# swesterfeld/audiowmark

Measured on AMD Instinct MI355X. Metric: audio seconds watermarked+decoded per wall-second (xRT), 44.1 kHz stereo, higher is better.
Workload: dtype f32; 1 GPU; 60 min stereo 44.1 kHz white noise per GPU resident in HBM, add+get incl. payload decode, payload 0123456789abcdef0011223344556677, strength 10; parallelism=1 GPU, patterns=108, payload_matches=104, ranks_seen=1

## Files before the change

audiowmark_amd/csrc/host/capi_kernels.cc:

```cpp
#include "context.hh"
#include "syncfinder.hh"
#include "wmget.hh"
#include "wmspeed.hh"
#include "utils.hh"
#include "wmfile.hh"
#include <atomic>
#include <future>
#include <thread>
#include <algorithm>
#include <cmath>
#include <cstdlib>
#include <cstring>
#include <memory>

using namespace awm;
namespace awm { Key capi_key (const uint8_t key[16]); }
namespace awm { extern int g_key_tables_on_device; int clip_key_tables_check (awm_ctx *ctx, const uint8_t *keys, size_t n_keys, long long mismatch_out[9]); }

namespace {

constexpr int LIMITER_BLOCK = Params::mark_sample_rate * int (Params::limiter_block_size_ms) / 1000;
const float LIMITER_CEILING = float (Params::limiter_ceiling);

constexpr int MAX_FRAMES_PER_BIT = 8;

int
check_ctx (awm_ctx *ctx)
{
  if (!ctx)
    {
      set_error ("null context");
      return AWM_ERR_ARG;
    }
  hipError_t e = hipSetDevice (ctx->device);
  if (e != hipSuccess)
    {
      set_error ("hipSetDevice: " + hip_error_string (e));
      return AWM_ERR_HIP;
    }
  if (params().frames_per_bit < 1 || params().frames_per_bit > MAX_FRAMES_PER_BIT || params().payload_size != 128)
    {
      set_error ("unsupported watermark parameters (frames_per_bit outside 1 .. 8 or a short payload)");
      return AWM_ERR_ARG;
    }
  return 0;
}

#define AWM_ENTER(ctx) \
  awm::ParamsBind params_bind__ ((ctx) ? (ctx)->own_params.get() : nullptr); \
  if (int rc__ = check_ctx (ctx)) return rc__

int
frames_per_span (awm_ctx *ctx, long long n_frames1024, int waves_per_simd = 0)
{
  static int cus = 0;
  if (!cus)
    {
      hipDeviceProp_t prop;
      cus = 256;
      if (hipGetDeviceProperties (&prop, ctx->device) == hipSuccess && prop.multiProcessorCount > 0)
        cus = prop.multiProcessorCount;
    }
  const int capacity = cus * 4 * (waves_per_simd > 0 ? waves_per_simd : awmk::add_mix_waves_per_simd());
  long long best_l = 4, best_cost = -1;
  for (int k = 1; k <= 16; k++)
    {
      long long l = (n_frames1024 + (long long) k * capacity - 1) / ((long long) k * capacity);
      l = std::max<long long> (l, 4);
      const long long cost = k * (l + 2);
      if (best_cost < 0 || cost < best_cost)
        {
          best_cost = cost;
          best_l = l;
        }
    }
  return int (std::min<long long> (best_l, 4096));
}

void
fill_pattern (const ResultSet::Pattern& p, awm_pattern& o)
{
  o.time = p.time;
  o.sync_index = p.sync_score.index;
  o.sync_quality = p.sync_score.quality;
  o.block_type = int (p.sync_score.block_type);
  o.type = int (p.type);
  o.decode_error = p.decode_error;
  o.speed = p.speed;
  o.n_bits = std::min<int> (p.bit_vec.size(), 128);
  for (int b = 0; b < o.n_bits; b++)
    o.bits[b] = p.bit_vec[b];
}

DeviceWav
make_wav (const float *pcm_d, size_t n_frames, int n_channels)
{
  DeviceWav w;
  w.data = pcm_d;
  w.n_frames = n_frames;
  w.n_channels = n_channels;
  w.sample_rate = Params::mark_sample_rate;
  return w;
}
// ... 96 lines not shown
{
  AWM_ENTER (ctx);
  if (!ctx->snr_on)
    {
      set_error ("awm_ctx_snr_end without awm_ctx_snr_begin");
      return AWM_ERR_ARG;
    }
  ctx->snr_on = false;
  double acc[2] = { 0, 0 };
  AWM_HIP_CHECK (hipDeviceSynchronize());
  AWM_HIP_CHECK (hipMemcpy (acc, ctx->ws_snr.ptr, sizeof (acc), hipMemcpyDeviceToHost));
  if (delta_power)
    *delta_power = acc[0];
  if (signal_power)
    *signal_power = acc[1];
  return 0;
}

int
awm_add_mix_d (awm_ctx *ctx, const float *pcm_in_d, float *out_d, size_t n_frames, int n_channels,
               const int8_t *frame_mod, double water_delta, size_t first_frame,
               const float *halo_before_d, const float *halo_after_d,
               float *block_max_d, size_t first_block, size_t n_blocks)
{
  AWM_ENTER (ctx);
  if (!pcm_in_d || !out_d || !frame_mod || n_channels < 1)
    {
      set_error ("awm_add_mix_d: bad argument");
      return AWM_ERR_ARG;
    }
  const size_t table_bytes = 2 * mark_block_frame_count() * Params::n_bands;
  if (int rc = ctx->ws_misc.reserve (table_bytes)) return rc;
  AWM_HIP_CHECK (hipMemcpyAsync (ctx->ws_misc.ptr, frame_mod, table_bytes, hipMemcpyHostToDevice, ctx->stream));
  return add_mix_impl (ctx, pcm_in_d, out_d, n_frames, n_channels, ctx->ws_misc.as<int8_t>(), water_delta, first_frame,
                       halo_before_d, halo_after_d, block_max_d, first_block, n_blocks);
}

int
awm_add_limit_d (awm_ctx *ctx, float *out_d, size_t n_frames, int n_channels, size_t first_sample,
                 const float *block_max_d, size_t first_block, size_t n_blocks)
{
  AWM_ENTER (ctx);
  const size_t tab_entries = awmk::limiter_tab_entries ((long long) n_frames, (long long) first_sample, LIMITER_BLOCK);
  if (int rc = ctx->ws_limit_tab.reserve ((tab_entries + 1) * sizeof (float2))) return rc;
  ProfScope ps (ctx, PROF_LIMITER, double (n_frames) * n_channels * 8.0);
  AWM_HIP_CHECK (awmk::launch_limiter (ctx->stream, out_d, (long long) n_frames, n_channels, (long long) first_sample, block_max_d,
                                       (long long) first_block, (long long) n_blocks, LIMITER_BLOCK, LIMITER_CEILING,
                                       ctx->ws_limit_tab.as<float2>(), tab_entries));
  return 0;
}

static int g_add_slab_mb = 0;
extern "C" void awm_debug_set_add_slab_mb (int mb) { g_add_slab_mb = mb < 0 ? 0 : mb; }

static bool
add_buffers_overlap (const float *in, const float *out, size_t n_values)
{
  const uintptr_t a = reinterpret_cast<uintptr_t> (in), b = reinterpret_cast<uintptr_t> (out), bytes = n_values * sizeof (float);
  return a < b + bytes && b < a + bytes;
}

static int
add_full (awm_ctx *ctx, const float *pcm_in_d, float *out_d, size_t n_frames, int n_channels,
          const int8_t *frame_mod_dev, double water_delta, int use_limiter, WorkLane *lane = nullptr, ReadyMarks *marks = nullptr)
{
  if (!lane)
    lane = ctx;
  if (marks)
    {
      marks->disarm();
      marks->base = out_d;
      marks->n_frames = n_frames;
    }
  hipStream_t st = lane->stream;
  float *block_max = nullptr;
  const size_t n_blocks = n_frames / LIMITER_BLOCK + 2;
  if (use_limiter)
    {
      if (int rc = lane->ws_block_max.reserve (n_blocks * sizeof (float))) return rc;
      block_max = lane->ws_block_max.as<float>();
      unsigned int bits;
      std::memcpy (&bits, &LIMITER_CEILING, sizeof (bits));
      AWM_HIP_CHECK (awmk::launch_fill_u32 (st, reinterpret_cast<unsigned int *> (block_max), bits, n_blocks));
    }
  const size_t FRAME = Params::frame_size;
  size_t slab = g_add_slab_mb ? (size_t (g_add_slab_mb) << 20) / (n_channels * sizeof (float)) / FRAME * FRAME : 0;
  if (!use_limiter || pcm_in_d == out_d || slab < 64 * FRAME || n_frames < 2 * slab)
    slab = 0;
  if (slab)
    {
      const size_t tab_entries = awmk::limiter_tab_entries ((long long) n_frames, 0, LIMITER_BLOCK);
      if (int rc = lane->ws_limit_tab.reserve ((tab_entries + 1) * sizeof (float2))) return rc;
      const size_t n_slabs = n_frames / slab;
      size_t limited = 0;
      for (size_t i = 0; i < n_slabs; i++)
        {
          const size_t a = i * slab, b = i + 1 == n_slabs ? n_frames : a + slab;
          if (int rc = add_mix_impl (ctx, pcm_in_d + a * n_channels, out_d + a * n_channels, b - a, n_channels, frame_mod_dev, water_delta,
                                     a / FRAME, a ? pcm_in_d + (a - FRAME) * n_channels : nullptr, b < n_frames ? pcm_in_d + b * n_channels : nullptr,
                                     block_max, 0, n_blocks, lane))
            return rc;
          const size_t upto = b == n_frames ? n_frames : (b / LIMITER_BLOCK >= 1 ? (b / LIMITER_BLOCK - 1) * size_t (LIMITER_BLOCK) : 0);
          if (upto > limited)
            {
              ProfScope ps (ctx, PROF_LIMITER, double (upto - limited) * n_channels * 8.0, st);
              AWM_HIP_CHECK (awmk::launch_limiter (st, out_d + limited * n_channels, (long long) (upto - limited), n_channels, (long long) limited, block_max, 0,
                                                   (long long) n_blocks, LIMITER_BLOCK, LIMITER_CEILING, lane->ws_limit_tab.as<float2>(), tab_entries));
              limited = upto;
            }
        }
      return 0;
    }
  if (int rc = add_mix_impl (ctx, pcm_in_d, out_d, n_frames, n_channels, frame_mod_dev, water_delta, 0, nullptr, nullptr,
                             block_max, 0, n_blocks, lane))
    return rc;
  std::vector<size_t> ends;
  if (marks)
    for (const ChunkRange& c : plan_chunks (n_frames, n_channels))
      {
        size_t e = std::min (n_frames, (c.first_frame + c.n_frames + LIMITER_BLOCK - 1) / LIMITER_BLOCK * size_t (LIMITER_BLOCK));
        if (e < n_frames && n_frames - e < size_t (LIMITER_BLOCK))
          e = n_frames;
        if (ends.empty() || e > ends.back())
          ends.push_back (e);
      }
// ... 614 lines not shown
  std::vector<size_t> idx (index, index + n_blocks);
  std::vector<std::vector<float>> raw;
  std::vector<char> okv;
  if (int rc = block_soft_bits (ctx, kt, make_wav (pcm_d, n_frames, n_channels), idx, raw, okv))
    return rc;
  const size_t n_bits = mark_data_frame_count() / params().frames_per_bit;
  for (size_t i = 0; i < n_blocks; i++)
    {
      ok[i] = okv[i];
      if (okv[i])
        std::copy (raw[i].begin(), raw[i].end(), out + i * n_bits);
      else
        std::fill (out + i * n_bits, out + (i + 1) * n_bits, 0.f);
    }
  return 0;
}

int
awm_viterbi_decode (awm_ctx *ctx, int block_type, const float *soft, size_t coded_len, size_t n, int *bits_out, float *error_out)
{
  AWM_ENTER (ctx);
  if (block_type < 0 || block_type > 2)
    return AWM_ERR_ARG;
  std::vector<std::vector<float>> in (n);
  for (size_t i = 0; i < n; i++)
    in[i].assign (soft + i * coded_len, soft + (i + 1) * coded_len);
  std::vector<std::vector<int>> bits;
  std::vector<float> errors;
  if (int rc = viterbi_decode (ctx, ConvBlockType (block_type), in, bits, errors))
    return rc;
  for (size_t i = 0; i < n; i++)
    {
      std::copy (bits[i].begin(), bits[i].end(), bits_out + i * bits[i].size());
      error_out[i] = errors[i];
    }
  return 0;
}

int
awm_add_watermark_d (awm_ctx *ctx, const uint8_t key[16], const char *payload_hex, const float *pcm_in_d, float *out_d,
                     size_t n_frames, int n_channels, int sample_rate)
{
  AWM_ENTER (ctx);
  if (n_channels >= 1 && add_buffers_overlap (pcm_in_d, out_d, n_frames * size_t (n_channels)))
    {
      set_error ("awm_add_watermark_d: the output overlaps the input");
      return AWM_ERR_ARG;
    }
  FrameModTable *fm = ctx->get_frame_mod (capi_key (key), payload_hex ? payload_hex : "");
  if (!fm)
    return AWM_ERR_ARG;
  if (sample_rate != Params::mark_sample_rate)
    return add_full_rate (ctx, pcm_in_d, out_d, n_frames, n_channels, fm->dev.as<int8_t>(), params().water_delta, !params().test_no_limiter, sample_rate);
  return add_full (ctx, pcm_in_d, out_d, n_frames, n_channels, fm->dev.as<int8_t>(), params().water_delta, !params().test_no_limiter);
}

static int g_add_payloads_fused = 1, g_add_payloads_fused_in_use = 0;
extern "C" void awm_debug_set_add_payloads_fused (int on) { g_add_payloads_fused = on; }
extern "C" int  awm_debug_add_payloads_fused_in_use (void) { return g_add_payloads_fused_in_use; }
extern "C" int  awm_debug_add_payloads_tile (void) { return awmk::ADD_MULTI_TILE; }

int
awm_add_watermark_payloads_d (awm_ctx *ctx, const uint8_t key[16], const char *const *payload_hex, size_t n_payloads,
                              const float *pcm_in_d, float *const *out_d, size_t n_frames, int n_channels, int sample_rate)
{
  AWM_ENTER (ctx);
  g_add_payloads_fused_in_use = 0;
  if (!n_payloads || !n_frames)
    return 0;
  if (!key || !payload_hex || !pcm_in_d || !out_d || n_channels < 1)
    {
      set_error ("awm_add_watermark_payloads_d: bad argument");
      return AWM_ERR_ARG;
    }
  if (ctx->snr_on)
    {
      set_error ("awm_add_watermark_payloads_d: not available while the SNR meter is armed (awm_ctx_snr_begin)");
      return AWM_ERR_ARG;
    }
  const size_t n_values = n_frames * size_t (n_channels);
  auto overlap = [n_values] (const float *a, const float *b) { return a < b + n_values && b < a + n_values; };
  for (size_t p = 0; p < n_payloads; p++)
    {
      if (!payload_hex[p] || !out_d[p])
        {
          set_error (string_printf ("awm_add_watermark_payloads_d: null pointer at index %zu", p));
          return AWM_ERR_ARG;
        }
      if (parse_payload (payload_hex[p]).empty())
        {
          set_error (string_printf ("awm_add_watermark_payloads_d: cannot parse payload '%s' at index %zu", payload_hex[p], p));
          return AWM_ERR_ARG;
        }
      if (overlap (out_d[p], pcm_in_d))
        {
          set_error (string_printf ("awm_add_watermark_payloads_d: output %zu overlaps the input", p));
          return AWM_ERR_ARG;
        }
      for (size_t q = 0; q < p; q++)
        if (overlap (out_d[p], out_d[q]))
          {
            set_error (string_printf ("awm_add_watermark_payloads_d: outputs %zu and %zu overlap", q, p));
            return AWM_ERR_ARG;
          }
    }
  const Key k = capi_key (key);
  const double water_delta = params().water_delta;
// ... 636 lines not shown
  };
  hipEvent_t ev_up[2] = { nullptr, nullptr };
  struct EvGuard { hipEvent_t (&ev)[2]; ~EvGuard() { for (hipEvent_t e : ev) if (e) (void) hipEventDestroy (e); } } guard { ev_up };
  for (auto& e : ev_up)
    AWM_HIP_CHECK (hipEventCreateWithFlags (&e, hipEventDisableTiming));
  std::vector<hipEvent_t> lane_done (2 * size_t (n_lanes), nullptr);
  struct DoneGuard { std::vector<hipEvent_t>& ev; ~DoneGuard() { for (hipEvent_t e : ev) if (e) (void) hipEventDestroy (e); } } done_guard { lane_done };
  for (auto& e : lane_done)
    AWM_HIP_CHECK (hipEventCreateWithFlags (&e, hipEventDisableTiming));
  int rc = 0, last_half = -1;
  std::future<bool> next_built;
  struct FutureGuard { std::future<bool>& f; ~FutureGuard() { if (f.valid()) f.wait(); } } future_guard { next_built };
  for (size_t s0 = 0, sidx = 0; s0 < n_clips && !rc; s0 += SUPER, sidx++)
    {
      const size_t sn = std::min (SUPER, n_clips - s0);
      const int half = int (sidx & 1);
      const bool built = next_built.valid() ? next_built.get() : build_super (s0, half);
      if (!built)
        {
          set_error ("frame_mod table of unexpected size");
          return AWM_ERR_GENERIC;
        }
      if (s0 + SUPER < n_clips)
        {
          if (sidx >= 1)
            AWM_HIP_CHECK (hipEventSynchronize (ev_up[half ^ 1]));
          next_built = std::async (std::launch::async, build_super, s0 + SUPER, half ^ 1);
        }
      int8_t *dev = ctx->ws_keytab.as<int8_t>() + size_t (half) * SUPER * table_bytes;
      if (sidx >= 2)
        for (int i = 1; i < n_lanes; i++)
          AWM_HIP_CHECK (hipStreamWaitEvent (ctx->stream, lane_done[size_t (half) * n_lanes + i], 0));
      AWM_HIP_CHECK (hipMemcpyAsync (dev, pin_base + size_t (half) * SUPER * table_bytes, sn * table_bytes, hipMemcpyHostToDevice, ctx->stream));
      AWM_HIP_CHECK (hipEventRecord (ev_up[half], ctx->stream));
      for (int i = 1; i < n_lanes; i++)
        AWM_HIP_CHECK (hipStreamWaitEvent (lanes[i]->stream, ev_up[half], 0));
      for (size_t i = 0; i < sn && !rc; i++)
        rc = add_full (ctx, pcm_in_d[s0 + i], out_d[s0 + i], n_frames[s0 + i], n_channels, dev + i * table_bytes, params().water_delta,
                       !params().test_no_limiter, lanes[(s0 + i) % n_lanes]);
      for (int i = 1; i < n_lanes && !rc; i++)
        AWM_HIP_CHECK (hipEventRecord (lane_done[size_t (half) * n_lanes + i], lanes[i]->stream));
      last_half = half;
    }
  if (last_half >= 0)
    AWM_HIP_CHECK (hipEventSynchronize (ev_up[last_half]));
  for (int i = 1; i < n_lanes; i++)
    {
      AWM_HIP_CHECK (hipEventRecord (lanes[i]->ev_sync, lanes[i]->stream));
      AWM_HIP_CHECK (hipStreamWaitEvent (ctx->stream, lanes[i]->ev_sync, 0));
    }
  return rc;
}

int
awm_get_watermark_d (awm_ctx *ctx, const uint8_t key[16], const float *pcm_d, size_t n_frames, int n_channels,
                     size_t max_out, awm_pattern *out)
{
  AWM_ENTER (ctx);
  ResultSet rs;
  if (int rc = get_watermark_device (ctx, { capi_key (key) }, make_wav (pcm_d, n_frames, n_channels), rs))
    return rc;
  for (size_t i = 0; i < rs.patterns.size() && i < max_out; i++)
    fill_pattern (rs.patterns[i], out[i]);
  return int (rs.patterns.size());
}


int
awm_get_watermark_keys_d (awm_ctx *ctx, const uint8_t *keys, int n_keys, const float *pcm_d, size_t n_frames, int n_channels,
                          size_t max_out, awm_pattern *out, int *key_of_pattern)
{
  AWM_ENTER (ctx);
  if (n_keys < 0 || (n_keys && !keys) || (max_out && !out))
    {
      set_error ("awm_get_watermark_keys_d: bad argument");
      return AWM_ERR_ARG;
    }
  const std::vector<Key> list = key_list_from (keys, n_keys);
  ResultSet rs;
  if (int rc = get_watermark_device (ctx, list, make_wav (pcm_d, n_frames, n_channels), rs))
    return rc;
  return fill_patterns_keys (rs, list, max_out, out, key_of_pattern);
}

int
awm_get_watermark_batch_d (awm_ctx *ctx, const uint8_t key[16], size_t n_clips, const float *const *pcm_d, const size_t *n_frames,
                           int n_channels, int n_threads, size_t max_out_per_clip, awm_pattern *out, int *n_out)
{
  AWM_ENTER (ctx);
  if (n_clips && (!pcm_d || !n_frames || !n_out || (max_out_per_clip && !out)))
    {
      set_error ("awm_get_watermark_batch_d: bad argument");
      return AWM_ERR_ARG;
    }
  std::vector<DeviceWav> clips;
  for (size_t i = 0; i < n_clips; i++)
    clips.push_back (make_wav (pcm_d[i], n_frames[i], n_channels));
  std::vector<ResultSet> sets;
  if (int rc = get_watermark_batch_device (ctx, { capi_key (key) }, clips, sets, n_threads))
    return rc;
  for (size_t i = 0; i < n_clips; i++)
    {
      n_out[i] = int (sets[i].patterns.size());
      for (size_t j = 0; j < sets[i].patterns.size() && j < max_out_per_clip; j++)
        fill_pattern (sets[i].patterns[j], out[i * max_out_per_clip + j]);
    }
  return 0;
}

int
awm_get_watermark_batch_keys_d (awm_ctx *ctx, const uint8_t *keys, size_t n_clips, const float *const *pcm_d, const size_t *n_frames,
                                int n_channels, int n_threads, size_t max_out_per_clip, awm_pattern *out, int *n_out)
{
  AWM_ENTER (ctx);
  if (n_clips && (!keys || !pcm_d || !n_frames || !n_out || (max_out_per_clip && !out)))
    {
      set_error ("awm_get_watermark_batch_keys_d: bad argument");
      return AWM_ERR_ARG;
    }
  std::vector<DeviceWav> clips;
  for (size_t i = 0; i < n_clips; i++)
    clips.push_back (make_wav (pcm_d[i], n_frames[i], n_channels));
  const std::vector<Key> clip_keys = key_list_from (keys, int (n_clips));
  std::vector<ResultSet> sets;
  if (int rc = get_watermark_batch_device (ctx, {}, clips, sets, n_threads, &clip_keys))
// ... 379 lines not shown
```

audiowmark_amd/csrc/host/capi_shard.cc:

```cpp
#include "context.hh"
#include "wmget.hh"
#include "utils.hh"
#include <algorithm>
#include <condition_variable>
#include <cstring>
#include <mutex>
#include <thread>

namespace awm {
Key capi_key (const uint8_t key[16]);
int sharded_plan_c (const uint64_t *span_frames, int world, size_t max_out, int *chunk, int *rank, uint64_t *first_sf, uint64_t *n_sf);
int sharded_add (awm_ctx *ctx, const Key& key, const std::string& payload_hex, const float *pcm_in, float *out, int C,
                 const uint64_t *span_frames, const awm_comm *comm);
int sharded_get (awm_ctx *ctx, const Key& key, const float *pcm, int C, const uint64_t *span_frames, const awm_comm *comm, ResultSet& result);
}

using namespace awm;

namespace {

int
enter (awm_ctx *ctx, const awm_comm *comm, const uint64_t *span_frames, int n_channels)
{
  if (!ctx || !comm || !span_frames || n_channels < 1 || comm->world < 1 || comm->rank < 0 || comm->rank >= comm->world
      || !comm->exchange_d || !comm->exchange_h || !comm->all_reduce_max_u32_d)
    {
      set_error ("awm_sharded_*: bad argument");
      return AWM_ERR_ARG;
    }
  if (hipSetDevice (ctx->device) != hipSuccess)
    {
      set_error ("hipSetDevice failed");
      return AWM_ERR_HIP;
    }
  if (params().frames_per_bit < 1 || params().frames_per_bit > 8 || params().payload_size != 128)
    {
      set_error ("unsupported watermark parameters (frames_per_bit outside 1 .. 8 or a short payload)");
      return AWM_ERR_ARG;
    }
  return 0;
}

void
fill_c_pattern (const ResultSet::Pattern& p, awm_pattern& o)
{
  o.time = p.time;
  o.sync_index = p.sync_score.index;
  o.sync_quality = p.sync_score.quality;
  o.block_type = int (p.sync_score.block_type);
  o.type = int (p.type);
  o.decode_error = p.decode_error;
  o.speed = p.speed;
  o.n_bits = std::min<int> (int (p.bit_vec.size()), 128);
  for (int b = 0; b < o.n_bits; b++)
    o.bits[b] = p.bit_vec[b];
}


struct LocalWorld
{
  int world;
  std::mutex mutex;
  std::condition_variable cond;
  int arrived = 0;
  unsigned long generation = 0;
  bool failed = false;
  struct Post { std::vector<const void *> ptr; std::vector<size_t> bytes; std::vector<int> to; bool device = false; };
  std::vector<Post> posts;
  std::vector<std::vector<uint32_t>> reduce;
  std::vector<int> device_of;
  explicit LocalWorld (int n) : world (n), posts (n), reduce (n), device_of (n, 0), active (n) {}
  int active;
  void
  barrier()
  {
    std::unique_lock<std::mutex> lock (mutex);
    const unsigned long gen = generation;
    arrived++;
    if (arrived >= active)
      {
        arrived = 0;
        generation++;
// ... 393 lines not shown
```

audiowmark_amd/csrc/host/capi_tables.cc:

```cpp
#include "context.hh"
#include "utils.hh"
#include "wmspeed.hh"
#include "random.hh"
#include <cstring>
#include <memory>

using namespace awm;

static Key
key_from_bytes (const uint8_t key[16])
{
  Key k;
  k.set_raw (key);
  return k;
}

namespace awm { Key capi_key (const uint8_t key[16]) { return key_from_bytes (key); } }

extern "C" {

int
awm_tab_up_down (const uint8_t key[16], int stream, int frame, int up[30], int down[30])
{
  UpDownGen gen (key_from_bytes (key), Random::Stream (stream));
// ... 208 lines not shown
      return AWM_ERR_ARG;
    }
  if (!(p->water_delta >= 0) || p->payload_size < 1 || p->frames_per_bit < 1 || p->get_n_best < 1 || !(p->get_chunk_size > 0))
    {
      set_error ("awm_params: value out of range");
      return AWM_ERR_ARG;
    }
  v.water_delta = p->water_delta;
  v.mix = p->mix != 0;
  v.hard = p->hard != 0;
  v.strict = p->strict != 0;
  v.snr = p->snr != 0;
  v.payload_size = size_t (p->payload_size);
  v.frames_per_bit = p->frames_per_bit;
  v.sync_threshold2 = p->sync_threshold2;
  v.get_n_best = p->get_n_best;
  v.get_chunk_size = p->get_chunk_size;
  v.detect_speed = p->detect_speed != 0;
  v.detect_speed_patient = p->detect_speed_patient != 0;
  v.try_speed = p->try_speed;
  v.test_speed = p->test_speed;
  v.test_cut = p->test_cut;
  v.test_no_sync = p->test_no_sync != 0;
  v.test_no_limiter = p->test_no_limiter != 0;
  v.test_truncate = p->test_truncate;
  return 0;
}

void
awm_params_init (awm_params *p)
{
  if (p)
    params_to_c (ParamValues(), p);
}

int
awm_set_global_params (const awm_params *p)
{
  ParamValues v = global_params();
  if (int rc = params_from_c (p, v))
    return rc;
  global_params() = v;
  return 0;
}

int
awm_ctx_set_params (awm_ctx *ctx, const awm_params *p)
{
  if (!ctx)
    {
      set_error ("null context");
      return AWM_ERR_ARG;
    }
  if (!p)
    {
      ctx->own_params.reset();
      return 0;
    }
  auto v = std::make_unique<ParamValues> (ctx->own_params ? *ctx->own_params : global_params());
  if (int rc = params_from_c (p, *v))
    return rc;
  ctx->own_params = std::move (v);
  return 0;
}

int
awm_ctx_get_params (const awm_ctx *ctx, awm_params *out)
{
  if (!out)
    return AWM_ERR_ARG;
  params_to_c (ctx && ctx->own_params ? *ctx->own_params : global_params(), out);
  return 0;
}

void
awm_set_quiet (int quiet)
{
  set_log_level (quiet ? Log::WARNING : Log::INFO);
}

}
```

audiowmark_amd/csrc/host/context.cc:

```cpp
#include "context.hh"
#include <algorithm>
#include <atomic>
#include <chrono>
#include <cstdlib>
#include "utils.hh"
#include <cmath>
#include <cstring>

namespace awm {

static thread_local std::string g_last_error;
void set_error (const std::string& msg) { g_last_error = msg; }
const std::string& last_error() { return g_last_error; }
std::string hip_error_string (hipError_t e) { return std::string (hipGetErrorName (e)) + " (" + hipGetErrorString (e) + ")"; }

static std::atomic<long>   g_dev_allocs { 0 }, g_pin_allocs { 0 };
static std::atomic<double> g_dev_alloc_ms { 0.0 }, g_pin_alloc_ms { 0.0 };
static void
note_alloc (std::atomic<long>& count, std::atomic<double>& ms, std::chrono::steady_clock::time_point t0)
{
  const double dt = std::chrono::duration<double, std::milli> (std::chrono::steady_clock::now() - t0).count();
  count.fetch_add (1, std::memory_order_relaxed);
  double cur = ms.load (std::memory_order_relaxed);
  while (!ms.compare_exchange_weak (cur, cur + dt, std::memory_order_relaxed))
// ... 654 lines not shown
  ctx->tabs.tw512d = reinterpret_cast<const double2 *> (ctx->tab_slide.as<double>() + off_tw512d);
  ctx->tabs.slide32 = reinterpret_cast<const float2 *> (ctx->tab_slide.as<double>() + off_slide32);
  if (int rc = upload (ctx->tab_mem, blob.data(), blob.size() * sizeof (float), ctx->stream))
    return rc;
  const float *base = ctx->tab_mem.as<float>();
  ctx->tabs.tw512 = reinterpret_cast<const float2 *> (base + off_tw512);
  ctx->tabs.tw1024 = reinterpret_cast<const float2 *> (base + off_tw1024);
  ctx->tabs.window = base + off_win;
  ctx->tabs.synth = base + off_synth;
  if (awmk::probe_dependent_launch_us (ctx->stream) < 0 && hipStreamSynchronize (ctx->stream) != hipSuccess)
    {
      set_error ("awm_ctx_create: the device does not complete work on the context's stream");
      return AWM_ERR_HIP;
    }
  *ctx_out = ctx.release();
  return 0;
}

int
awm_ctx_set_chunk_lanes (awm_ctx *ctx, int n_lanes)
{
  if (!ctx || n_lanes < 1)
    return AWM_ERR_ARG;
  ctx->chunk_lanes = std::min (n_lanes, awm::CHUNK_LANES);
  return 0;
}

int
awm_ctx_warm_up (awm_ctx *ctx, int detect_speed, int file_level)
{
  if (!ctx)
    return AWM_ERR_ARG;
  AWM_HIP_CHECK (hipSetDevice (ctx->device));
  const int lanes = std::max (1, std::min (ctx->chunk_lanes, awm::CHUNK_LANES)) * (detect_speed ? 2 : 1);
  for (int i = 0; i < lanes && i < awm::MAX_LANES; i++)
    if (!ctx->lane (i))
      {
        awm::set_error ("cannot create a work lane (stream)");
        return AWM_ERR_HIP;
      }
  if (file_level && !ctx->get_copy_stream())
    {
      awm::set_error ("cannot create the copy stream");
      return AWM_ERR_HIP;
    }
  return 0;
}

int
awm_ctx_trim (awm_ctx *ctx)
{
  if (!ctx)
    return AWM_ERR_ARG;
  AWM_HIP_CHECK (hipSetDevice (ctx->device));
  AWM_HIP_CHECK (hipStreamSynchronize (ctx->stream));
  for (auto& l : ctx->extra_lanes)
    if (l)
      {
        if (l->stream)
          AWM_HIP_CHECK (hipStreamSynchronize (l->stream));
        l->release_lane();
      }
  if (ctx->copy_stream)
    AWM_HIP_CHECK (hipStreamSynchronize (ctx->copy_stream));
  ctx->release_lane();
  ctx->file_staging.release();
  awm::speed_workspace_free (ctx);
  ctx->ws_add_batch.release();
  ctx->pin_add_batch.release();
  ctx->ws_merge_soft.release();
  ctx->ws_rate_a.release();
  ctx->ws_rate_b.release();
  ctx->ws_rate_c.release();
  for (awm_ctx *h : ctx->helpers)
    if (h && h != ctx)
      if (int rc = awm_ctx_trim (h)) return rc;
  return 0;
}

void
awm_ctx_destroy (awm_ctx *ctx)
{
  if (!ctx)
    return;
  (void) hipSetDevice (ctx->device);
  (void) hipStreamSynchronize (ctx->stream);
  for (auto& kt : ctx->key_tables)
    release_key_tables (*kt);
  for (auto& t : ctx->frame_mod_tables)
    t->dev.release();
  for (auto& t : ctx->resample_tables)
    t->ctab.release();
  awm::speed_workspace_free (ctx);
  ctx->ws_snr.release();
  ctx->ws_add_batch.release();
  ctx->pin_add_batch.release();
  if (ctx->ev_add_batch)
    (void) hipEventDestroy (ctx->ev_add_batch);
  ctx->ev_add_batch = nullptr;
  ctx->ws_merge_soft.release();
  for (hipEvent_t e : ctx->merge_events)
    if (e)
      (void) hipEventDestroy (e);
  ctx->merge_events.clear();
  ctx->ws_rate_a.release();
  ctx->ws_rate_b.release();
  ctx->ws_rate_c.release();
  ctx->tab_mem.release();
  ctx->tab_slide.release();
  for (auto& l : ctx->extra_lanes)
    if (l)
      {
        if (l->stream)
          (void) hipStreamSynchronize (l->stream);
        l->release_lane();
        if (l->own_stream && l->stream)
          (void) hipStreamDestroy (l->stream);
      }
  ctx->release_lane();
  if (ctx->copy_stream)
    (void) hipStreamSynchronize (ctx->copy_stream);
  ctx->file_staging.release();
  ctx->ready.release();
  if (ctx->copy_stream)
    (void) hipStreamDestroy (ctx->copy_stream);
  if (ctx->own_stream && ctx->stream)
    (void) hipStreamDestroy (ctx->stream);
  delete ctx;
}

int awm_ctx_device (const awm_ctx *ctx) { return ctx ? ctx->device : -1; }

int
awm_ctx_synchronize (awm_ctx *ctx)
{
  if (!ctx)
    return AWM_ERR_ARG;
  AWM_HIP_CHECK (hipStreamSynchronize (ctx->stream));
  return 0;
}

void *awm_ctx_stream (awm_ctx *ctx) { return ctx ? (void *) ctx->stream : nullptr; }

int
awm_ctx_set_stream (awm_ctx *ctx, void *hip_stream)
{
  if (!ctx)
    return AWM_ERR_ARG;
  AWM_HIP_CHECK (hipStreamSynchronize (ctx->stream));
  if (ctx->own_stream && ctx->stream)
    (void) hipStreamDestroy (ctx->stream);
  ctx->stream = (hipStream_t) hip_stream;
  ctx->own_stream = false;
  return 0;
}

}
```

audiowmark_amd/csrc/host/context.hh:

```
#pragma once
#include <condition_variable>
#include <mutex>
#include <hip/hip_runtime.h>
#include <map>
#include <mutex>
#include <memory>
#include <string>
#include <vector>
#include "../hip/kernels.hh"
#include "wmcommon.hh"

namespace awm { void set_error (const std::string& msg); const std::string& last_error(); std::string hip_error_string (hipError_t e); }

#define AWM_HIP_CHECK(expr) \
  do { hipError_t e__ = (expr); if (e__ != hipSuccess) { awm::set_error (std::string (#expr) + ": " + awm::hip_error_string (e__)); return AWM_ERR_HIP; } } while (0)

namespace awm {

inline void
cpu_relax()
{
  for (int k = 0; k < 48; k++)
    __builtin_ia32_pause();
}
// ... 74 lines not shown
  int        slice_want_n = 0;
  const int *want_of_slice (int i) const { return slice_want_flat ? slice_want_flat + size_t (i) * slice_want_n : slice_want[i].data(); }
  int        want_rows_of_slices() const { return slice_want_flat ? slice_want_n : int (slice_want[0].size()); }
};

struct ClipKeyHost
{
  std::vector<unsigned>      chains;
  std::vector<int>           row_frames;
  std::vector<int>           want;
  std::vector<int>           perm;
  std::vector<unsigned char> pos;
  MixTable                   mix;
  std::vector<int>           inv_order;
};
ClipKeyHost build_clip_key_host (const Key& key);

struct ResampleTable
{
  int       rate_in = 0, rate_out = 0;
  int       hl = 0, np = 0, step = 0;
  DevBuffer ctab;
};

std::vector<float> zita_table (double frel, unsigned hl, unsigned np);
int upload_sync (DevBuffer& buf, const void *src, size_t bytes, hipStream_t st);

struct SpeedWorkspace;
struct SpeedScratch;
struct WorkLane;
void speed_scratch_free (WorkLane *lane);
} struct awm_ctx; namespace awm {
void speed_workspace_free (awm_ctx *ctx);

struct FileStaging
{
  static constexpr int RING = 4;
  PinnedBuffer in_host[RING], out_host[RING];
  DevBuffer    in_dev[RING], out_dev[RING];
  DevBuffer    pcm;
  bool         keep = false;
  size_t       kept_values = 0;
  int          kept_channels = 0, kept_rate = 0;
  hipEvent_t   in_copied[RING] = {}, in_used[RING] = {}, out_encoded[RING] = {}, out_copied[RING] = {};
  bool         have_events = false;
  bool         ensure_events();
  void         release();
};

struct ReadyMarks
{
  const float *base = nullptr;
  size_t       n_frames = 0;
  bool         armed = false;
  std::vector<std::pair<size_t, hipEvent_t>> marks;
  std::vector<hipEvent_t> pool;
  size_t       used = 0;
  hipEvent_t   next_event();
  bool         live = false, live_done = false;
  std::mutex   mu;
  std::condition_variable cv;
  void         disarm() { armed = false; live = live_done = false; marks.clear(); used = 0; base = nullptr; n_frames = 0; }
  void         release();
};

struct FrameModTable
{
  std::vector<unsigned char> key;
  std::string payload;
  bool        mix = true;
  int         frames_per_bit = 2;
  unsigned long last_use = 0;
  DevBuffer   dev;
};

}

namespace awm {
enum ProfId { PROF_ADD_MIX, PROF_LIMITER, PROF_SYNC_DB, PROF_SYNC_SCAN, PROF_LOCAL_MEAN, PROF_REFINE_DB, PROF_REFINE_SCAN,
              PROF_BLOCK_DB, PROF_SOFT_BITS, PROF_VITERBI, PROF_STFT,
              PROF_RESAMPLE, PROF_RESAMPLE_VAR, PROF_SPEED_MAGS, PROF_SPEED_COMPARE, PROF_KEYTAB, PROF_ADD_MIX_MULTI, PROF_COUNT };
struct ProfPending { int id; hipEvent_t start, stop; };
}

namespace awm {
struct WorkLane
{
  hipStream_t    stream = nullptr;
  bool           own_stream = false;
  DevBuffer ws_db, ws_block_db, ws_have, ws_q, ws_raw, ws_mean, ws_misc, ws_refine, ws_refine_have, ws_soft,
            ws_viterbi, ws_viterbi_in, ws_viterbi_bits, ws_viterbi_err, ws_viterbi_sync, ws_block_max, ws_clip, ws_idx, ws_limit_tab, ws_jobs, ws_group, ws_keytab, ws_keytab_aux, ws_keytab_scratch;
  DevBuffer ws_shard_edge, ws_shard_tail, ws_shard_q;
  PinnedBuffer pin_refine_in[2], pin_refine_q[2], pin_peaks, pin_blocks, pin_jobs, pin_bits, pin_small, pin_group, pin_shard, pin_shard_up, pin_keytab;
  hipEvent_t   ev_refine[2] = { nullptr, nullptr };
  hipEvent_t   ev_sync = nullptr;
  SpeedScratch *speed_scratch = nullptr;
  double       prof_live_fraction = 1.0;
  unsigned int *viterbi_sync (size_t n_decodes);
  void release_lane();
};
constexpr int MAX_LANES = 16;
constexpr int CHUNK_LANES = 4;
}

struct awm_ctx : awm::WorkLane
{
  int            device = -1;
  awmk::DevTables tabs {};
  awm::DevBuffer tab_mem, tab_slide;

  std::vector<std::unique_ptr<awm::KeyTables>>     key_tables;
  std::vector<std::unique_ptr<awm::FrameModTable>> frame_mod_tables;
  std::vector<std::unique_ptr<awm::ResampleTable>> resample_tables;
  awm::ResampleTable *get_resample_table (int rate_in, int rate_out);
  awm::DevBuffer ws_rate_a, ws_rate_b, ws_rate_c;
// ... 69 lines not shown
```

audiowmark_amd/csrc/host/wmget.cc:

```cpp
#include "wmget.hh"
#include "wmdecode.hh"
#include "wmspeed.hh"
#include <atomic>
#include <future>
#include <chrono>
#include <memory>
#include <thread>
#include "utils.hh"
#include <algorithm>
#include <cmath>
#include <map>

namespace awm {
int g_key_tables_on_device = 1;


std::vector<float>
normalize_soft_bits (const std::vector<float>& soft_bits)
{
  std::vector<float> norm;
  norm.reserve (soft_bits.size());
  if (params().hard)
    {
      for (float v : soft_bits)
// ... 457 lines not shown
  }
};

}

void
combine_blocks (const std::vector<PatternRawBits>& raw_blocks, const DeviceWav& wav, size_t chunk, std::vector<PendingDecode>& pending)
{
  const BlockList list { raw_blocks, (long long) (mark_block_frame_count() * Params::frame_size) };
  for (size_t pos = 0; pos < raw_blocks.size(); pos++)
    {
      const PatternRawBits& b = raw_blocks[pos];
      if (b.block_type != ConvBlockType::b)
        continue;
      const size_t partner = list.nearest (0, pos, ConvBlockType::a, (long long) b.index - list.block_len, Params::frame_size / 2);
      if (partner == NO_BLOCK)
        continue;
      const PatternRawBits& a = raw_blocks[partner];
      const SyncFinder::Score score { b.index, (a.quality + b.quality) / 2, ConvBlockType::ab };
      pending.push_back ({ ConvBlockType::ab, 1, { { a.slot, 0 }, { b.slot, 1 } }, 0, 0, double (b.index) / wav.sample_rate, score,
                           ResultSet::Type::BLOCK, chunk });
    }
  std::vector<size_t> best;
  float best_sum = 0;
  for (size_t start = 0; start < raw_blocks.size(); start++)
    {
      std::vector<size_t> chain = list.chain_from (start);
      const float sum = list.quality_sum (chain);
      if (sum > best_sum)
        {
          best = std::move (chain);
          best_sum = sum;
        }
    }
  if (best.size() < 2)
    return;
  PendingDecode all { ConvBlockType::ab, 2, {}, 0, 0, 0.0, { 0, 0, ConvBlockType::a }, ResultSet::Type::ALL, chunk };
  for (size_t pos : best)
    {
      const PatternRawBits& blk = raw_blocks[pos];
      const int ab = blk.block_type == ConvBlockType::b;
      all.src.push_back ({ blk.slot, ab });
      (ab ? all.norm1 : all.norm0)++;
      all.score.quality += blk.quality;
    }
  all.score.quality /= all.norm0 + all.norm1;
  pending.push_back (std::move (all));
}

int g_merge_decodes = 0;
extern "C" void awm_debug_set_merge_decodes (int on) { g_merge_decodes = on; }
int g_chunk_stagger = -1;
extern "C" void awm_debug_set_chunk_stagger (int on) { g_chunk_stagger = on; }
int g_speed_overlap = 1;
extern "C" void awm_debug_set_speed_overlap (int on) { g_speed_overlap = on; }
namespace {

int
block_decoder_run (awm_ctx *ctx, WorkLane *home, bool spread, const std::vector<Key>& key_list, const DeviceWav& stream,
                   const std::vector<ChunkRange>& chunks, const std::vector<ResultSet *>& result_sets, double speed,
                   std::string *debug_sync_first_chunk, int lane_base = 0)
{
  const size_t count = mark_block_frame_count();
  std::vector<SyncFinder::Score> first_scores;
  const int n_lanes = !spread ? 1 : int (std::min<size_t> (chunks.size(), size_t (std::max (1, std::min (ctx->chunk_lanes, CHUNK_LANES)))));
  std::vector<WorkLane *> lanes;
  if (!spread)
    lanes.push_back (home);
  else
    for (int i = 0; i < std::max (n_lanes, 1); i++)
      {
        WorkLane *l = ctx->lane (lane_base + i);
        if (!l)
          {
            set_error ("cannot create a work lane (stream)");
            return AWM_ERR_HIP;
          }
        lanes.push_back (l);
      }
  ReadyMarks *marks = (spread && lane_base == 0 && lanes.size() > 1 && ctx->ready.armed && ctx->ready.base == stream.data
                       && ctx->ready.n_frames == stream.n_frames && (ctx->ready.live || !ctx->ready.marks.empty())) ? &ctx->ready : nullptr;
  if (marks && !marks->live)
    std::rotate (lanes.begin(), lanes.begin() + 1, lanes.end());
  else if (lanes.size() > 1 && lane_base == 0)
    {
      if (!ctx->ev_sync)
        AWM_HIP_CHECK (hipEventCreateWithFlags (&ctx->ev_sync, hipEventDisableTiming));
      AWM_HIP_CHECK (hipEventRecord (ctx->ev_sync, ctx->stream));
      for (size_t i = 1; i < lanes.size(); i++)
        AWM_HIP_CHECK (hipStreamWaitEvent (lanes[i]->stream, ctx->ev_sync, 0));
    }
  auto wait_for_mark = [&] (WorkLane *lane, size_t last_sample_plus_one) -> int {
    if (!marks)
      return 0;
    if (marks->live)
      {
        std::unique_lock<std::mutex> lock (marks->mu);
        marks->cv.wait (lock, [&] { return marks->live_done || (!marks->marks.empty() && marks->marks.back().first >= last_sample_plus_one); });
        hipEvent_t ev = nullptr;
        for (const auto& m : marks->marks)
          if (m.first >= last_sample_plus_one)
            {
              ev = m.second;
              break;
            }
        if (!ev && !marks->marks.empty())
          ev = marks->marks.back().second;
        lock.unlock();
        if (ev)
          AWM_HIP_CHECK (hipStreamWaitEvent (lane->stream, ev, 0));
        return 0;
      }
    if (lane->stream == ctx->stream)
      return 0;
    for (const auto& m : marks->marks)
      if (m.first >= last_sample_plus_one)
        {
          AWM_HIP_CHECK (hipStreamWaitEvent (lane->stream, m.second, 0));
          return 0;
        }
    AWM_HIP_CHECK (hipStreamWaitEvent (lane->stream, marks->marks.back().second, 0));
    return 0;
  };
  struct LaneDrain
  {
    const std::vector<WorkLane *>& lanes;
    bool ok = false;
    ~LaneDrain()
    {
      if (!ok)
        for (WorkLane *l : lanes)
          (void) hipStreamSynchronize (l->stream);
    }
  } drain { lanes };
  auto chunk_wav = [&] (size_t c) {
    DeviceWav cw = stream;
// ... 1334 lines not shown
```

include/awm_hip.h:

```cpp
#ifndef AWM_HIP_H
#define AWM_HIP_H

#include <stddef.h>
#include <stdint.h>

#ifdef __cplusplus
extern "C" {
#endif

#define AWM_ERR_GENERIC    (-1)
#define AWM_ERR_NO_DEVICE  (-2)
#define AWM_ERR_ARG        (-3)
#define AWM_ERR_HIP        (-4)
#define AWM_ERR_IO         (-5)

#define AWM_FRAME_SIZE      1024
#define AWM_N_BANDS         81
#define AWM_BLOCK_FRAMES    2226
#define AWM_SOFT_BITS       858

typedef struct awm_ctx awm_ctx;

const char *awm_last_error (void);
const char *awm_version (void);
// ... 154 lines not shown
                     const uint64_t *span_frames, size_t max_out, awm_pattern *out);

int awm_multi_add_watermark_batch_d (awm_ctx *const *ctxs, int n_ctx, const int *ctx_of_clip, const uint8_t *keys, const uint8_t *one_key,
                                     const char *payload_hex, size_t n_clips, const float *const *pcm_in_d, float *const *out_d,
                                     const size_t *n_frames, int n_channels);
int awm_multi_get_watermark_batch_d (awm_ctx *const *ctxs, int n_ctx, const int *ctx_of_clip, const uint8_t *keys, const uint8_t *one_key,
                                     size_t n_clips, const float *const *pcm_d, const size_t *n_frames, int n_channels,
                                     size_t max_out_per_clip, awm_pattern *out, int *n_out);

int awm_ctx_set_helpers (awm_ctx *ctx, awm_ctx *const *helpers, int n_helpers);

void awm_set_speed_params (int detect_speed, int detect_speed_patient, double try_speed, double test_speed);
size_t awm_resample_ratio_frames (size_t n_frames, int n_channels, int rate, double ratio, double max_in_seconds);
int awm_resample_ratio_d (awm_ctx *ctx, const float *pcm_in_d, size_t n_frames, int n_channels, int rate, double ratio,
                          double max_in_seconds, float *out_d, size_t n_out_frames);
int awm_detect_speed_d (awm_ctx *ctx, const uint8_t key[16], const float *pcm_d, size_t n_frames, int n_channels, int rate,
                        int patient, double *speed_out, double *quality_out);
int awm_speed_clip_location_d (awm_ctx *ctx, const uint8_t key[16], const float *pcm_d, size_t n_frames, int n_channels, int rate,
                               double seconds, int candidates, double *location);
int awm_speed_mags_d (awm_ctx *ctx, const uint8_t key[16], const float *pcm_d, size_t n_frames, int n_channels, int rate,
                      double clip_location, double center, double seconds, size_t max_rows, float *out);
int awm_speed_scan_d (awm_ctx *ctx, const uint8_t key[16], const float *pcm_d, size_t n_frames, int n_channels, int rate,
                      double clip_location, double seconds, double step, int n_steps, int n_center_steps,
                      const double *speeds, int n_speeds, size_t max_out, double *out_speed, double *out_quality);

int    awm_speed_select_n_best (double *speed, double *quality, int count, int n);
double awm_speed_smooth_best (const double *speed, const double *quality, int count, double step, double distance);
size_t awm_speed_clip_positions (const uint8_t key[16], size_t n_values, size_t max_out, uint64_t *positions);
int    awm_speed_clip_candidates (const uint8_t key[16], const float *hashed_values, size_t n, int candidates, double *locations);

void awm_debug_set_viterbi_super (int on);
void awm_debug_set_viterbi_persistent (int on);
double awm_debug_dependent_launch_us (void);
int  awm_debug_viterbi_one_launch_in_use (void);
void awm_debug_set_sliding3 (int on);
void awm_debug_set_refine_form (int form);
int  awm_debug_refine_form (void);
void awm_debug_set_k4s_ablate (int flags);
int  awm_debug_sync_db_sliding_d (awm_ctx *ctx, const float *pcm_d, size_t n_frames, int n_channels, const long long *base_d, size_t n_streams,
                                  int count, int ld, float *out_d);
void awm_debug_set_soft_bits_generic (int on);
void awm_debug_set_chunk_stagger (int mode);
void awm_debug_set_resample_phase (int on);
void awm_debug_set_get_overlap (int on);
void awm_debug_set_speed_compare_wide (int on);
void awm_debug_set_speed_compare_fold (int on);
void awm_debug_set_resample_var_mode (int mode);
void awm_debug_set_speed_overlap (int on);
int  awm_debug_frame_mod_tables_d (awm_ctx *ctx, const uint8_t *keys, size_t n_keys, const char *payload_hex, int8_t *tables_out);
int  awm_debug_clip_key_tables_check_d (awm_ctx *ctx, const uint8_t *keys, size_t n_keys, long long mismatch_out[9]);
void awm_debug_set_key_tables_on_device (int on);
void awm_debug_set_merge_decodes (int on);
void awm_debug_set_add_batched (int on);
void awm_debug_set_add_slab_mb (int mb);
void awm_debug_set_add_payloads_fused (int on);
int  awm_debug_add_payloads_fused_in_use (void);
int  awm_debug_add_payloads_tile (void);
void awm_debug_set_fft_pair (int on);
void awm_debug_set_clip_poison (int on);
void awm_debug_set_clip_pad_margin (int frames);
void awm_debug_set_staged_threads (int n);
void awm_debug_clip_key_timing (double us_out[3]);
double awm_debug_time_group_key_tables (int n_keys, int threads);
void awm_debug_set_group_fallback (int on);
void awm_debug_alloc_stats (long *dev_allocs, double *dev_ms, long *pinned_allocs, double *pinned_ms);
void awm_debug_file_timing (double ms_out[8]);
void awm_debug_set_io_flags (int flags);

void awm_set_io_threads (int n);

void awm_set_quiet (int quiet);

void awm_set_params (double water_delta, int mix, int frames_per_bit, int test_no_limiter,
                     double sync_threshold2, int n_best, double chunk_size_min);
typedef struct
{
  size_t struct_size;
  double water_delta;
  int    mix;
  int    hard;
  int    strict;
  int    snr;
  int    payload_size;
  int    frames_per_bit;
  double sync_threshold2;
  int    get_n_best;
  double get_chunk_size;
  int    detect_speed, detect_speed_patient;
  double try_speed, test_speed;
  int    test_cut, test_no_sync, test_no_limiter, test_truncate;
} awm_params;
void awm_params_init (awm_params *p);
int  awm_set_global_params (const awm_params *p);
int  awm_ctx_set_params (awm_ctx *ctx, const awm_params *p);
int  awm_ctx_get_params (const awm_ctx *ctx, awm_params *out);

int  awm_ctx_snr_begin (awm_ctx *ctx);
int  awm_ctx_snr_end (awm_ctx *ctx, double *signal_power, double *delta_power);

#ifdef __cplusplus
}
#endif
#endif
```

Before: 751,700 xRT.

## Hand per-chunk ready marks from add_watermark to a following get

```diff
diff --git a/audiowmark_amd/csrc/host/capi_kernels.cc b/audiowmark_amd/csrc/host/capi_kernels.cc
--- a/audiowmark_amd/csrc/host/capi_kernels.cc
+++ b/audiowmark_amd/csrc/host/capi_kernels.cc
@@ -46,9 +46,12 @@
   return 0;
 }
 
-#define AWM_ENTER(ctx) \
+#define AWM_ENTER_KEEP_MARKS(ctx) \
   awm::ParamsBind params_bind__ ((ctx) ? (ctx)->own_params.get() : nullptr); \
   if (int rc__ = check_ctx (ctx)) return rc__
+#define AWM_ENTER(ctx) \
+  AWM_ENTER_KEEP_MARKS (ctx); \
+  (ctx)->ready.drop_add_marks()
 
 int
 frames_per_span (awm_ctx *ctx, long long n_frames1024, int waves_per_simd = 0)
@@ -251,6 +254,8 @@
 
 static int g_add_slab_mb = 0;
 extern "C" void awm_debug_set_add_slab_mb (int mb) { g_add_slab_mb = mb < 0 ? 0 : mb; }
+static int g_add_marks = 1;
+extern "C" void awm_debug_set_add_marks (int on) { g_add_marks = on; }
 
 static bool
 add_buffers_overlap (const float *in, const float *out, size_t n_values)
@@ -270,6 +275,7 @@
       marks->disarm();
       marks->base = out_d;
       marks->n_frames = n_frames;
+      marks->n_channels = n_channels;
     }
   hipStream_t st = lane->stream;
   float *block_max = nullptr;
@@ -990,7 +996,12 @@
     return AWM_ERR_ARG;
   if (sample_rate != Params::mark_sample_rate)
     return add_full_rate (ctx, pcm_in_d, out_d, n_frames, n_channels, fm->dev.as<int8_t>(), params().water_delta, !params().test_no_limiter, sample_rate);
-  return add_full (ctx, pcm_in_d, out_d, n_frames, n_channels, fm->dev.as<int8_t>(), params().water_delta, !params().test_no_limiter);
+  const bool hand_over = g_add_marks && !g_add_slab_mb && n_frames > 0 && plan_chunks (n_frames, n_channels).size() > 1;
+  const int rc = add_full (ctx, pcm_in_d, out_d, n_frames, n_channels, fm->dev.as<int8_t>(), params().water_delta, !params().test_no_limiter, nullptr,
+                           hand_over ? &ctx->ready : nullptr);
+  if (rc)
+    ctx->ready.disarm();
+  return rc;
 }
 
 static int g_add_payloads_fused = 1, g_add_payloads_fused_in_use = 0;
@@ -1733,11 +1744,28 @@
   return rc;
 }
 
+extern "C++" {
+namespace {
+struct MarksUse
+{
+  awm_ctx *ctx;
+  MarksUse (awm_ctx *c, const float *pcm_d, size_t n_frames, int n_channels) : ctx (c)
+  {
+    ReadyMarks& rm = ctx->ready;
+    if (!(rm.armed && !rm.live && rm.base == pcm_d && rm.n_frames == n_frames && rm.n_channels == n_channels))
+      rm.disarm();
+  }
+  ~MarksUse() { ctx->ready.disarm(); }
+};
+}
+}
+
 int
 awm_get_watermark_d (awm_ctx *ctx, const uint8_t key[16], const float *pcm_d, size_t n_frames, int n_channels,
                      size_t max_out, awm_pattern *out)
 {
-  AWM_ENTER (ctx);
+  AWM_ENTER_KEEP_MARKS (ctx);
+  MarksUse marks_use (ctx, pcm_d, n_frames, n_channels);
   ResultSet rs;
   if (int rc = get_watermark_device (ctx, { capi_key (key) }, make_wav (pcm_d, n_frames, n_channels), rs))
     return rc;
@@ -1751,7 +1779,8 @@
 awm_get_watermark_keys_d (awm_ctx *ctx, const uint8_t *keys, int n_keys, const float *pcm_d, size_t n_frames, int n_channels,
                           size_t max_out, awm_pattern *out, int *key_of_pattern)
 {
-  AWM_ENTER (ctx);
+  AWM_ENTER_KEEP_MARKS (ctx);
+  MarksUse marks_use (ctx, pcm_d, n_frames, n_channels);
   if (n_keys < 0 || (n_keys && !keys) || (max_out && !out))
     {
       set_error ("awm_get_watermark_keys_d: bad argument");
diff --git a/audiowmark_amd/csrc/host/capi_shard.cc b/audiowmark_amd/csrc/host/capi_shard.cc
--- a/audiowmark_amd/csrc/host/capi_shard.cc
+++ b/audiowmark_amd/csrc/host/capi_shard.cc
@@ -28,6 +28,7 @@
       set_error ("awm_sharded_*: bad argument");
       return AWM_ERR_ARG;
     }
+  ctx->ready.drop_add_marks();
   if (hipSetDevice (ctx->device) != hipSuccess)
     {
       set_error ("hipSetDevice failed");
diff --git a/audiowmark_amd/csrc/host/capi_tables.cc b/audiowmark_amd/csrc/host/capi_tables.cc
--- a/audiowmark_amd/csrc/host/capi_tables.cc
+++ b/audiowmark_amd/csrc/host/capi_tables.cc
@@ -284,6 +284,7 @@
       set_error ("null context");
       return AWM_ERR_ARG;
     }
+  ctx->ready.drop_add_marks();
   if (!p)
     {
       ctx->own_params.reset();
diff --git a/audiowmark_amd/csrc/host/context.cc b/audiowmark_amd/csrc/host/context.cc
--- a/audiowmark_amd/csrc/host/context.cc
+++ b/audiowmark_amd/csrc/host/context.cc
@@ -730,6 +730,7 @@
 {
   if (!ctx)
     return AWM_ERR_ARG;
+  ctx->ready.drop_add_marks();
   AWM_HIP_CHECK (hipSetDevice (ctx->device));
   AWM_HIP_CHECK (hipStreamSynchronize (ctx->stream));
   for (auto& l : ctx->extra_lanes)
@@ -814,6 +815,7 @@
 {
   if (!ctx)
     return AWM_ERR_ARG;
+  ctx->ready.drop_add_marks();
   AWM_HIP_CHECK (hipStreamSynchronize (ctx->stream));
   return 0;
 }
@@ -825,6 +827,7 @@
 {
   if (!ctx)
     return AWM_ERR_ARG;
+  ctx->ready.drop_add_marks();
   AWM_HIP_CHECK (hipStreamSynchronize (ctx->stream));
   if (ctx->own_stream && ctx->stream)
     (void) hipStreamDestroy (ctx->stream);
diff --git a/audiowmark_amd/csrc/host/context.hh b/audiowmark_amd/csrc/host/context.hh
--- a/audiowmark_amd/csrc/host/context.hh
+++ b/audiowmark_amd/csrc/host/context.hh
@@ -150,6 +150,7 @@
 {
   const float *base = nullptr;
   size_t       n_frames = 0;
+  int          n_channels = 0;
   bool         armed = false;
   std::vector<std::pair<size_t, hipEvent_t>> marks;
   std::vector<hipEvent_t> pool;
@@ -158,7 +159,8 @@
   bool         live = false, live_done = false;
   std::mutex   mu;
   std::condition_variable cv;
-  void         disarm() { armed = false; live = live_done = false; marks.clear(); used = 0; base = nullptr; n_frames = 0; }
+  void         drop_add_marks() { if (armed && !live) disarm(); }
+  void         disarm() { armed = false; live = live_done = false; marks.clear(); used = 0; base = nullptr; n_frames = 0; n_channels = 0; }
   void         release();
 };
 
diff --git a/audiowmark_amd/csrc/host/wmget.cc b/audiowmark_amd/csrc/host/wmget.cc
--- a/audiowmark_amd/csrc/host/wmget.cc
+++ b/audiowmark_amd/csrc/host/wmget.cc
@@ -533,6 +533,8 @@
 extern "C" void awm_debug_set_merge_decodes (int on) { g_merge_decodes = on; }
 int g_chunk_stagger = -1;
 extern "C" void awm_debug_set_chunk_stagger (int on) { g_chunk_stagger = on; }
+std::atomic<long> g_add_marks_used { 0 };
+extern "C" long awm_debug_add_marks_used (void) { return g_add_marks_used.load(); }
 int g_speed_overlap = 1;
 extern "C" void awm_debug_set_speed_overlap (int on) { g_speed_overlap = on; }
 namespace {
@@ -560,9 +562,13 @@
         lanes.push_back (l);
       }
   ReadyMarks *marks = (spread && lane_base == 0 && lanes.size() > 1 && ctx->ready.armed && ctx->ready.base == stream.data
-                       && ctx->ready.n_frames == stream.n_frames && (ctx->ready.live || !ctx->ready.marks.empty())) ? &ctx->ready : nullptr;
+                       && ctx->ready.n_frames == stream.n_frames && (!ctx->ready.n_channels || ctx->ready.n_channels == stream.n_channels)
+                       && (ctx->ready.live || !ctx->ready.marks.empty())) ? &ctx->ready : nullptr;
   if (marks && !marks->live)
-    std::rotate (lanes.begin(), lanes.begin() + 1, lanes.end());
+    {
+      std::rotate (lanes.begin(), lanes.begin() + 1, lanes.end());
+      g_add_marks_used++;
+    }
   else if (lanes.size() > 1 && lane_base == 0)
     {
       if (!ctx->ev_sync)
diff --git a/include/awm_hip.h b/include/awm_hip.h
--- a/include/awm_hip.h
+++ b/include/awm_hip.h
@@ -230,6 +230,8 @@
 void awm_debug_set_key_tables_on_device (int on);
 void awm_debug_set_merge_decodes (int on);
 void awm_debug_set_add_batched (int on);
+void awm_debug_set_add_marks (int on);
+long awm_debug_add_marks_used (void);
 void awm_debug_set_add_slab_mb (int mb);
 void awm_debug_set_add_payloads_fused (int on);
 int  awm_debug_add_payloads_fused_in_use (void);
```

Result: no change. 749,500 xRT (-0.3%).
